# xshazwar/noize-job

Measured on AMD Instinct MI355X. Metric: Mcells/s 4096^2 simplex13oct->Gauss5x17->FlowMap->Erosion; %HBM roofline @1/8GPU, higher is better.
Workload: dtype f32

## Files before the change

noize_job_amd/csrc/nz_filter.hip:

```cpp
#include <cstdlib>

#include "nz_internal.hpp"
#include "nz_chain_plan.hpp"

namespace {

constexpr int CT = 256;
constexpr int TW = 128;
__host__ __device__ constexpr int conv_hx(int H) { return (H + 3) & ~3; }
constexpr int TH = 64;

__device__ __forceinline__ int clampi(int v, int lo, int hi) { return v < lo ? lo : (v > hi ? hi : v); }

__device__ __forceinline__ int xcd_tile_index() {
    int bid = blockIdx.x;
    int nb = gridDim.x, q = nb >> 3, r = nb & 7;
    int x = bid & 7, k = bid >> 3;
    return x * q + (x < r ? x : r) + k;
}

__device__ __forceinline__ void tile_origin(const nz_geom &g, int OW, int OH, int &ox0, int &oz0) {
    int tiles_x = (g.cols + OW - 1) / OW;
    int bid = xcd_tile_index();
    int by = bid / tiles_x;
// ... 42 lines not shown
__device__ __forceinline__ void store16_sc1(float *base, size_t float_off, float4 v) {
    __amdgpu_buffer_rsrc_t r = __builtin_amdgcn_make_buffer_rsrc(base, 0, -1, 0x00020000);
    nz_v4u t = {__float_as_uint(v.x), __float_as_uint(v.y), __float_as_uint(v.z), __float_as_uint(v.w)};
    __builtin_amdgcn_raw_buffer_store_b128(t, r, (int)(float_off * 4), 0, NZ_AUX_SC1);
}
__device__ __forceinline__ float load4_sc1(const float *base, size_t float_off) {
    __amdgpu_buffer_rsrc_t r = __builtin_amdgcn_make_buffer_rsrc(const_cast<float *>(base), 0, -1, 0x00020000);
    return __uint_as_float(__builtin_amdgcn_raw_buffer_load_b32(r, (int)(float_off * 4), 0, NZ_AUX_SC1));
}
__device__ __forceinline__ void store4_sc1(float *base, size_t float_off, float v) {
    __amdgpu_buffer_rsrc_t r = __builtin_amdgcn_make_buffer_rsrc(base, 0, -1, 0x00020000);
    __builtin_amdgcn_raw_buffer_store_b32(__float_as_uint(v), r, (int)(float_off * 4), 0, NZ_AUX_SC1);
}

template <bool FAST>
__device__ __forceinline__ float tap_acc(float total, float v, float k) {
    return FAST ? __builtin_fmaf(v, k, total) : total + v * k;
}
template <bool FAST, bool SEED>
__device__ __forceinline__ float tap_first(float v, float k) {
    return FAST ? __builtin_fmaf(v, k, 0.0f) : SEED ? 0.0f + v * k : v * k;
}

template <int KS, bool UNIT, int NT, bool SC1, bool FAST, int RBT>
__device__ __forceinline__ void conv_tile(const float *__restrict__ src, float *__restrict__ dst, const nz_geom &g,
                                          const nz_kernel_taps &taps, int T, int aligned, int ox0, int oz0,
                                          float4 *s_edge_raw NZ_PB_PARAM) {
    constexpr int O = (KS - 1) / 2;
    constexpr int WN = 4 + 2 * O;
    constexpr int ZN = RBT + 2 * O;
    constexpr int TH = NT / 32 * RBT;
    static_assert(O <= RBT, "a block's window reaches into the neighbouring blocks only");
    constexpr int NBUF = conv_nbuf(O);
    float4 (*s_edge)[TH / RBT][2][O][TW / 4] = reinterpret_cast<float4 (*)[TH / RBT][2][O][TW / 4]>(s_edge_raw);

    const int tid = threadIdx.x, cg = tid & 31, rb = tid >> 5;
    const int H = T * O, HX = conv_hx(H);
    const int OW = TW - 2 * HX, OH = TH - 2 * H;
    const int lx0 = ox0 - HX, lz0 = oz0 - H;
    const int gx0 = lx0 + cg * 4, gzb = lz0 + rb * RBT;
    const bool inside = lx0 >= 0 && lx0 + TW <= g.cols && lz0 >= g.zc0 && lz0 + TH - 1 <= g.zc1;
    const bool fast = inside && aligned;
    const bool edge16 = !inside && aligned && (g.cols & 3) == 0;
    NZ_PROBE_T(0);
    NZ_PROBE(14, (unsigned long long)__builtin_amdgcn_s_getreg(4 | (0 << 6) | (31 << 11)));
    NZ_PROBE(15, (unsigned long long)__builtin_amdgcn_s_getreg(20 | (0 << 6) | (31 << 11)));

    float v[RBT][4];
    if (fast) {
#pragma unroll
        for (int r = 0; r < RBT; r++) {
            float4 t = SC1 ? load16_sc1(src, (size_t)(gzb + r) * g.pitch + gx0)
                           : *reinterpret_cast<const float4 *>(src + (size_t)(gzb + r) * g.pitch + gx0);
            v[r][0] = t.x; v[r][1] = t.y; v[r][2] = t.z; v[r][3] = t.w;
        }
// ... 8 lines not shown
            v[r][0] = t.x; v[r][1] = t.y; v[r][2] = t.z; v[r][3] = t.w;
        }
        asm volatile("; 16-byte edge loads issued" ::: "memory");
    } else {
        asm volatile("; clamped 4-byte loads of an edge tile" ::: "memory");
#pragma unroll
        for (int r = 0; r < RBT; r++) {
            size_t row = (size_t)clampi(gzb + r, g.zc0, g.zc1) * g.pitch;
#pragma unroll
            for (int e = 0; e < 4; e++) {
                const size_t off = row + clampi(gx0 + e, 0, g.cols - 1);
                v[r][e] = SC1 ? load4_sc1(src, off) : src[off];
            }
        }
    }
    if constexpr (SC1) __builtin_amdgcn_s_setprio(0);
#ifdef NZ_CONV_PROBE
    asm volatile("s_waitcnt vmcnt(0)" ::: "memory");
    NZ_PROBE_T(9);
#endif
    const int icx = g.cols - 1 - gx0 + O;
    const int iz0 = g.zc0 - gzb + O, iz1 = g.zc1 - gzb + O;

    for (int t = 0; t < T; t++) {
#pragma unroll
        for (int r = 0; r < RBT; r++) {
            float w[WN];
#pragma unroll
            for (int o = 0; o < O; o++) {
                w[o] = dpp_prev(v[r][4 - O + o]);
                w[4 + O + o] = dpp_next(v[r][o]);
            }
#pragma unroll
            for (int e = 0; e < 4; e++) w[O + e] = v[r][e];
            if (!inside) {
                if (gx0 == 0) {
#pragma unroll
                    for (int o = 0; o < O; o++) w[o] = w[O];
                }
                if (icx >= O && icx < WN - 1) {
                    float wc = w[O];
#pragma unroll
                    for (int i = O + 1; i < WN; i++) wc = (i == icx) ? w[i] : wc;
#pragma unroll
                    for (int i = O + 1; i < WN; i++) w[i] = (i > icx) ? wc : w[i];
                }
            }
#pragma unroll
            for (int e = 0; e < 4; e++) {
// ... 28 lines not shown
            for (int e = 0; e < 4; e++) z[O + r][e] = v[r][e];
        if (!inside) {
            if (iz0 > 0 && iz0 < ZN) {
#pragma unroll
                for (int e = 0; e < 4; e++) {
                    float c = z[0][e];
#pragma unroll
                    for (int i = 1; i < ZN; i++) c = (i == iz0) ? z[i][e] : c;
#pragma unroll
                    for (int i = 0; i < ZN - 1; i++) z[i][e] = (i < iz0) ? c : z[i][e];
                }
            }
            if (iz1 >= 0 && iz1 < ZN - 1) {
#pragma unroll
                for (int e = 0; e < 4; e++) {
                    float c = z[0][e];
#pragma unroll
                    for (int i = 1; i < ZN; i++) c = (i == iz1) ? z[i][e] : c;
#pragma unroll
                    for (int i = 1; i < ZN; i++) z[i][e] = (i > iz1) ? c : z[i][e];
                }
            }
        }
#pragma unroll
        for (int r = 0; r < RBT; r++) {
#pragma unroll
            for (int e = 0; e < 4; e++) {
                float total = tap_first<FAST, !UNIT>(z[r + 2 * O][e], taps.kz[0]);
#pragma unroll
                for (int kk = 1; kk < KS; kk++) total = tap_acc<FAST>(total, z[r + 2 * O - kk][e], taps.kz[kk]);
                v[r][e] = UNIT ? total : total * taps.factor;
            }
        }
        NZ_PROBE_T(1 + t);
    }

    if constexpr (UNIT && !FAST) {
#pragma unroll
        for (int r = 0; r < RBT; r++)
#pragma unroll
            for (int e = 0; e < 4; e++) v[r][e] += 0.0f;
    }

    if constexpr (SC1) __builtin_amdgcn_s_setprio(3);
    if (fast) {
#pragma unroll
        for (int r = 0; r < RBT; r++) {
            int lr = rb * RBT + r, gz = gzb + r;
// ... 13 lines not shown
                if (SC1) store16_sc1(dst, (size_t)gz * g.pitch + gx0, make_float4(v[r][0], v[r][1], v[r][2], v[r][3]));
                else *reinterpret_cast<float4 *>(dst + (size_t)gz * g.pitch + gx0) = make_float4(v[r][0], v[r][1], v[r][2], v[r][3]);
            }
        }
    } else {
        asm volatile("; guarded stores of an edge tile" ::: "memory");
#pragma unroll
        for (int r = 0; r < RBT; r++) {
            int lr = rb * RBT + r, gz = gzb + r;
            bool in = lr >= H && lr < H + OH && cg * 4 >= HX && cg * 4 < HX + OW && gz < g.or1 && gx0 < g.cols;
            if (in) {
#pragma unroll
                for (int e = 0; e < 4; e++)
                    if (gx0 + e < g.cols) {
                        if (SC1) store4_sc1(dst, (size_t)gz * g.pitch + gx0 + e, v[r][e]);
                        else dst[(size_t)gz * g.pitch + gx0 + e] = v[r][e];
                    }
            }
        }
    }
    NZ_PROBE_T(12);
}

template <int KS, bool UNIT, int NT, bool FAST, int RBT>
__global__ __launch_bounds__(NT) __attribute__((amdgpu_waves_per_eu(conv_waves(KS, NT, RBT)))) void conv_reg_kernel(const float *__restrict__ src, float *__restrict__ dst, nz_geom g,
                                                     nz_kernel_taps taps, int T, int aligned) {
    constexpr int O = (KS - 1) / 2;
    constexpr int TH = NT / 32 * RBT;
    constexpr int NBUF = conv_nbuf(O);
    __shared__ float4 s_edge[NBUF][TH / RBT][2][O][TW / 4];
    const int H = T * O, HX = conv_hx(H);
    src += blockIdx.y * g.bstride;
    dst += blockIdx.y * g.bstride;
    int ox0, oz0;
    tile_origin(g, TW - 2 * HX, TH - 2 * H, ox0, oz0);
    NZ_PB_INIT;
    conv_tile<KS, UNIT, NT, false, FAST, RBT>(src, dst, g, taps, T, aligned, ox0, oz0, &s_edge[0][0][0][0][0] NZ_PB_ARG);
}

typedef int nz_v8i __attribute__((ext_vector_type(8)));
static_assert(sizeof(nz_v8i) == sizeof(nz_chain_item) && offsetof(nz_chain_item, stride) == 28, "a record is loaded as eight dwords");
struct nz_chain {
    const nz_chain_item *items;
    unsigned epoch;
    int *flags;
    float *plane[2];
    int delay_item, delay_sleeps;
    int spin_limit;
    unsigned *err_host;
    unsigned *err_epoch;
};

template <int KS, bool UNIT, int NT, bool FAST, int RBT>
__global__ __launch_bounds__(NT) __attribute__((amdgpu_waves_per_eu(conv_waves(KS, NT, RBT)))) void conv_chain_kernel(nz_geom g, nz_kernel_taps taps,
                                                                                                                       nz_chain ch, int aligned) {
    constexpr int O = (KS - 1) / 2;
    constexpr int TH = NT / 32 * RBT;
    constexpr int NBUF = conv_nbuf(O);
    __shared__ float4 s_edge[NBUF][TH / RBT][2][O][TW / 4];
    NZ_PB_INIT;
    NZ_PROBE_T(18);
    const nz_v8i rec = *reinterpret_cast<const nz_v8i *>(ch.items + blockIdx.x);
    __builtin_amdgcn_s_setprio(3);
    const nz_chain_item it = {rec[0], rec[1], rec[2], rec[3], rec[4], rec[5], rec[6], rec[7]};
    const int l = it.tl >> 16, T = it.tl & 0xffff;
    NZ_PROBE_T(7);
    NZ_PROBE(13, ((unsigned long long)l << 32) | (unsigned)(it.item));
    {
        const int tid = threadIdx.x, dr = tid >= 6 ? 2 : tid >= 3 ? 1 : 0, dc = tid - 3 * dr;
        if (tid < 9 && dr < it.ny && dc < it.nx) {
            const int *f = ch.flags + it.dep0 + dr * it.stride + dc;
            int spins = 0;
            while ((unsigned)__hip_atomic_load(f, __ATOMIC_RELAXED, __HIP_MEMORY_SCOPE_AGENT) != ch.epoch) {
                __builtin_amdgcn_s_sleep(32);
                if (++spins > ch.spin_limit) {
                    atomicMin(ch.err_epoch, ch.epoch);
                    __threadfence();
                    __hip_atomic_store(ch.err_host, 1u, __ATOMIC_RELEASE, __HIP_MEMORY_SCOPE_SYSTEM);
                    break;
                }
            }
        }
        if (it.ny > 0) __syncthreads();
    }
    NZ_PROBE_T(8);
    if (it.item == ch.delay_item)
        for (int i = 0; i < ch.delay_sleeps; i++) __builtin_amdgcn_s_sleep(127);
    conv_tile<KS, UNIT, NT, true, FAST, RBT>(ch.plane[l & 1], ch.plane[(l + 1) & 1], g, taps, T, aligned, it.ox0, it.oz0, &s_edge[0][0][0][0][0] NZ_PB_ARG);
    asm volatile("s_waitcnt vmcnt(0)" ::: "memory");
    NZ_PROBE_T(10);
    __syncthreads();
    NZ_PROBE_T(11);
    if (threadIdx.x == 0) {
        __hip_atomic_store(&ch.flags[it.item], (int)ch.epoch, __ATOMIC_RELAXED, __HIP_MEMORY_SCOPE_AGENT);
    }
}



template <int E>
__global__ __launch_bounds__(CT) void erosion_reg_kernel(const float *__restrict__ src, float *__restrict__ dst,
                                                        nz_geom g, int aligned) {
    __shared__ float4 s_edge[TH / RB][E][TW / 4];
    constexpr float BIG = 3.40282347e+38f;
    constexpr int HX = E > 4 ? 8 : 4;
    static_assert(E >= 1 && E <= RB, "the window reaches one 8-row block / two lanes back at most");
    const int tid = threadIdx.x, cg = tid & 31, rb = tid >> 5;
    const int OW = TW - HX, OH = TH - E;
    src += blockIdx.y * g.bstride;
    dst += blockIdx.y * g.bstride;
    int ox0, oz0;
// ... 292 lines not shown
static conv_shape conv_shape_of(int ksize, const nz_geom &g) {
    if (!conv_small_grid(ksize, g)) return CONV_BIG;
    return ksize == 5 && (long long)g.cols * (g.or1 - g.or0) * g.count <= CONV_TINY_CELLS ? CONV_TINY : CONV_SMALL;
}

template <int KS, class F>
auto with_conv_shape(conv_shape sh, F &&f) {
    using std::integral_constant;
    if constexpr (KS == 5)
        if (sh == CONV_TINY) return f(integral_constant<int, CONV_TINY_NT>(), integral_constant<int, CONV_TINY_RB>());
    if (sh != CONV_BIG) return f(integral_constant<int, CONV_SMALL_NT>(), integral_constant<int, CONV_SMALL_RB>());
    return f(integral_constant<int, (KS >= 5 ? 512 : 256)>(), integral_constant<int, RB>());
}

struct conv_tiling { int x, y; };
template <int KS, int NT, int RBT>
conv_tiling conv_tiles(const nz_geom &g, int T) {
    constexpr int O = (KS - 1) / 2, RTH = NT / 32 * RBT;
    const int H = T * O, HX = conv_hx(H);
    const int OW = TW - 2 * HX, OH = RTH - 2 * H;
    return {(g.cols + OW - 1) / OW, (g.or1 - g.or0 + OH - 1) / OH};
}

template <int KS, int NT, int RBT>
int32_t launch_fused_nt(hipStream_t s, const float *src, float *dst, const nz_geom &g, const nz_kernel_taps &k, int T) {
    const conv_tiling t = conv_tiles<KS, NT, RBT>(g, T);
    const long long blocks = (long long)t.x * t.y;
    int aligned = ((reinterpret_cast<uintptr_t>(src) | reinterpret_cast<uintptr_t>(dst) | (uintptr_t)(g.pitch * 4)) & 15) == 0;
    nz_with_unit_fast(k, [&](auto unit, auto fast) {
        NZ_LAUNCH((conv_reg_kernel<KS, unit, NT, fast, RBT>), dim3((unsigned)blocks, g.count), dim3(NT), 0, s, src, dst, g, k, T, aligned);
    });
    NZ_HIP(hipGetLastError());
    return NZ_OK;
}

template <int KS>
int32_t launch_fused(hipStream_t s, const float *src, float *dst, const nz_geom &g, const nz_kernel_taps &k, int T) {
    return with_conv_shape<KS>(conv_shape_of(KS, g), [&](auto nt, auto rbt) { return launch_fused_nt<KS, nt, rbt>(s, src, dst, g, k, T); });
}

int g_chain_delay_item = -1, g_chain_delay_sleeps = 0;
int g_chain_spin_limit = 1 << 21;

template <int KS, int NT, int RBT>
int32_t launch_chain_nt(hipStream_t s, float *plane0, float *plane1, const nz_geom &g, const nz_kernel_taps &k,
                        const nz_chain_item *items, int total, int *flags, unsigned epoch, unsigned *err_host, unsigned *err_epoch) {
    nz_chain ch{};
    ch.items = items;
    ch.epoch = epoch;
    ch.flags = flags;
    ch.plane[0] = plane0;
    ch.plane[1] = plane1;
    ch.delay_item = g_chain_delay_item;
    ch.delay_sleeps = g_chain_delay_sleeps;
    ch.spin_limit = g_chain_spin_limit;
    ch.err_host = err_host;
    ch.err_epoch = err_epoch;
    int aligned = ((reinterpret_cast<uintptr_t>(plane0) | reinterpret_cast<uintptr_t>(plane1) | (uintptr_t)(g.pitch * 4)) & 15) == 0;
    nz_with_unit_fast(k, [&](auto unit, auto fast) {
        NZ_LAUNCH((conv_chain_kernel<KS, unit, NT, fast, RBT>), dim3((unsigned)total), dim3(NT), 0, s, g, k, ch, aligned);
    });
    NZ_HIP(hipGetLastError());
    return NZ_OK;
}

template <int KS>
int32_t launch_chain(hipStream_t s, float *plane0, float *plane1, const nz_geom &g, const nz_kernel_taps &k,
                     const nz_chain_item *items, int total, int *flags, unsigned epoch, unsigned *err_host, unsigned *err_epoch) {
    return with_conv_shape<KS>(conv_shape_of(KS, g), [&](auto nt, auto rbt) {
        return launch_chain_nt<KS, nt, rbt>(s, plane0, plane1, g, k, items, total, flags, epoch, err_host, err_epoch);
    });
}

}

bool nz_conv_small_grid(int ksize, const nz_geom &g) { return conv_small_grid(ksize, g); }
bool nz_conv_tiny_grid(int ksize, const nz_geom &g) { return conv_shape_of(ksize, g) == CONV_TINY; }

bool nz_conv_chain_key(int ksize, const nz_geom &g, const int *Ts, int L, nz_chain_key *key) {
    if (L < 1 || L > NZ_CHAIN_MAXL || (ksize != 3 && ksize != 5 && ksize != 7 && ksize != 9)) return false;
    for (int l = 0; l < L; l++)
        if (Ts[l] < 1 || Ts[l] > nz_conv_max_fused(ksize)) return false;
    const conv_shape sh = conv_shape_of(ksize, g);
// ... 149 lines not shown
```

noize_job_amd/csrc/nz_flow_common.hpp:

```cpp
#pragma once

#include "nz_internal.hpp"

namespace {

constexpr float TIMESTEP = 0.2f;

__device__ __forceinline__ int clampi(int v, int lo, int hi) { return v < lo ? lo : (v > hi ? hi : v); }

struct flux4 {
    float w, e, s, n;
};

__device__ __forceinline__ flux4 compute_flow(float totalHt, float water_0, float tW, float tE, float tS, float tN,
                                              flux4 old) {
    float dW = totalHt - tW, dE = totalHt - tE, dS = totalHt - tS, dN = totalHt - tN;
    flux4 f;
    f.w = fmaxf(0.0f, old.w + dW);
    f.e = fmaxf(0.0f, old.e + dE);
    f.s = fmaxf(0.0f, old.s + dS);
    f.n = fmaxf(0.0f, old.n + dN);
    float sum_ = (f.w + f.e) + (f.s + f.n);
    if (sum_ > 0.0f) {
        float K = water_0 / (sum_ * TIMESTEP);
        K = fmaxf(0.0f, fminf(1.0f, K));
        f.w *= K; f.e *= K; f.s *= K; f.n *= K;
    } else {
        f.w = 0.0f; f.e = 0.0f; f.s = 0.0f; f.n = 0.0f;
    }
    return f;
}

__device__ __forceinline__ flux4 compute_flow_nb(float totalHt, float water_0, float tW, float tE, float tS, float tN,
                                                 flux4 old) {
    float dW = totalHt - tW, dE = totalHt - tE, dS = totalHt - tS, dN = totalHt - tN;
    flux4 f;
    f.w = fmaxf(0.0f, old.w + dW);
    f.e = fmaxf(0.0f, old.e + dE);
    f.s = fmaxf(0.0f, old.s + dS);
    f.n = fmaxf(0.0f, old.n + dN);
    float sum_ = (f.w + f.e) + (f.s + f.n);
    float K = water_0 / (sum_ * TIMESTEP);
    K = fmaxf(0.0f, fminf(1.0f, K));
    f.w *= K; f.e *= K; f.s *= K; f.n *= K;
    return f;
}

__device__ __forceinline__ float update_water(float water, flux4 own, float fE_west, float fW_east, float fN_south,
                                              float fS_north) {
    float flowOUT = own.w + own.e + own.s + own.n;
    float flowIN = 0.0f;
    flowIN += fE_west;
    flowIN += fW_east;
    flowIN += fN_south;
    flowIN += fS_north;
    float ht = water + ((flowIN - flowOUT) * TIMESTEP);
    return fmaxf(0.0f, ht);
}


template <bool FAST>
__device__ __forceinline__ flux4 compute_flow_m(float totalHt, float water_0, float tW, float tE, float tS, float tN, flux4 old,
                                                bool branch_free) {
    if (!FAST) return branch_free ? compute_flow_nb(totalHt, water_0, tW, tE, tS, tN, old) : compute_flow(totalHt, water_0, tW, tE, tS, tN, old);
    float dW = totalHt - tW, dE = totalHt - tE, dS = totalHt - tS, dN = totalHt - tN;
    flux4 f;
    f.w = fmaxf(0.0f, old.w + dW);
    f.e = fmaxf(0.0f, old.e + dE);
    f.s = fmaxf(0.0f, old.s + dS);
    f.n = fmaxf(0.0f, old.n + dN);
    float sum_ = (f.w + f.e) + (f.s + f.n);
    float K = water_0 * __builtin_amdgcn_rcpf(sum_ * TIMESTEP);
    K = fmaxf(0.0f, fminf(1.0f, K));
    f.w *= K; f.e *= K; f.s *= K; f.n *= K;
    return f;
}

template <bool FAST>
__device__ __forceinline__ float update_water_m(float water, flux4 own, float fE_west, float fW_east, float fN_south,
                                                float fS_north) {
    if (!FAST) return update_water(water, own, fE_west, fW_east, fN_south, fS_north);
    float flowOUT = own.w + own.e + own.s + own.n;
    float flowIN = ((fE_west + fW_east) + fN_south) + fS_north;
    return fmaxf(0.0f, __builtin_fmaf(flowIN - flowOUT, TIMESTEP, water));
}

template <bool FAST>
__device__ __forceinline__ float velocity_norm_m(float dl, float dr, float dt, float db, float nmin, float nrange, float inv_range) {
    const float vx = (dl + dr) * 0.5f;
    const float vy = (dt + db) * 0.5f;
    if (!FAST) {
        float v = sqrtf(vx * vx + vy * vy);
        if (nrange < 1e-12f) v = 0.0f;
        return (v - nmin) / nrange;
    }
    float v = __builtin_amdgcn_sqrtf(__builtin_fmaf(vx, vx, vy * vy));
    if (nrange < 1e-12f) v = 0.0f;
    return (v - nmin) * inv_range;
}

constexpr int FT_MAX_N = 5;

}
```

noize_job_amd/csrc/nz_flow_stream.hip:

```cpp
#include <cstdlib>

#include "nz_internal.hpp"
#include "nz_flow_common.hpp"

namespace {

__device__ __forceinline__ float wave_prev0(float v) {
    return __builtin_bit_cast(float, __builtin_amdgcn_mov_dpp(__builtin_bit_cast(int, v), 0x138, 0xf, 0xf, true));
}
__device__ __forceinline__ float wave_next0(float v) {
    return __builtin_bit_cast(float, __builtin_amdgcn_mov_dpp(__builtin_bit_cast(int, v), 0x130, 0xf, 0xf, true));
}

#ifdef NZ_FLOW_PROBE
__device__ unsigned long long *nz_flow_probe_buf = nullptr;
#define NZ_FPROBE(slot, val)                                                                                        \
    do {                                                                                                            \
        if (threadIdx.x == 0 && nz_flow_probe_buf)                                                                  \
            nz_flow_probe_buf[((size_t)blockIdx.y * gridDim.x + blockIdx.x) * 8 + (slot)] = (val);                  \
    } while (0)
#else
#define NZ_FPROBE(slot, val)
#endif
constexpr int FS_WPE = 2;
// ... 50 lines not shown
        if (i == NACT - 1) ring[((t + 2) & (FS_RING - 1)) * 64] = hn;
        const bool fa = !COND || (r >= b.loF[i] && r < b.hiF[i]);
        if (fa) {
            float left = wave_prev0(st.T0[i][NC - 1]), right = wave_next0(st.T0[i][0]);
            if (XEDGE) {
                left = lane_x0 ? st.T0[i][0] : left;
                right = lane_x1 ? st.T0[i][NC - 1] : right;
            }
#pragma unroll
            for (int e = 0; e < NC; e++) {
                const float self = st.T0[i][e];
                const float tW = e == 0 ? left : st.T0[i][e > 0 ? e - 1 : 0];
                float tE = e == NC - 1 ? right : st.T0[i][e + 1 < NC ? e + 1 : e];
                if (XEDGE && NC == 2 && e == 0 && lane_x1o) tE = self;
                float tS = st.Tm[i][e], tN = Tp[e];
                if (COND) {
                    if (r <= g.zc0) tS = self;
                    if (r >= g.zc1) tN = self;
                }
                flux4 old;
                if (i == 0) old = flux4{0.0f, 0.0f, 0.0f, 0.0f};
                else old = flux4{st.FA[i > 0 ? i - 1 : 0][e][0], st.FA[i > 0 ? i - 1 : 0][e][1],
                                 st.FA[i > 0 ? i - 1 : 0][e][2], st.FA[i > 0 ? i - 1 : 0][e][3]};
                const flux4 f = compute_flow_m<FAST>(self, st.W0[i][e], tW, tE, tS, tN, old, true);
                FC[e][0] = f.w; FC[e][1] = f.e; FC[e][2] = f.s; FC[e][3] = f.n;
            }
        } else {
#pragma unroll
            for (int e = 0; e < NC; e++)
#pragma unroll
                for (int k = 0; k < 4; k++) FC[e][k] = 0.0f;
        }
        if (i > 0) {
#pragma unroll
            for (int e = 0; e < NC; e++)
#pragma unroll
                for (int k = 0; k < 4; k++) {
                    st.FA[i > 0 ? i - 1 : 0][e][k] = st.FB[i > 0 ? i - 1 : 0][e][k];
                    st.FB[i > 0 ? i - 1 : 0][e][k] = FCprev[e][k];
                }
        }
        const int rw = r - 1;
        const bool wa = !COND || (rw >= b.loW[i] && rw < b.hiW[i]);
        float Wn[NC], Tn[NC];
#pragma unroll
        for (int e = 0; e < NC; e++) Wn[e] = Tn[e] = 0.0f;
        if (wa) {
// ... 265 lines not shown
```

noize_job_amd/csrc/nz_fractal.hip:

```cpp
#include <cstdlib>

#include "nz_internal.hpp"

namespace {

__device__ __forceinline__ float fracf_(float x) { return x - floorf(x); }
__device__ __forceinline__ float lerpf_(float a, float b, float s) { return a + s * (b - a); }
__device__ __forceinline__ float stepf_(float y, float x) { return x >= y ? 1.0f : 0.0f; }
__device__ __forceinline__ float mod289f(float x) { return x - floorf(x * (1.0f / 289.0f)) * 289.0f; }
__device__ __forceinline__ float mod7f(float x) { return x - floorf(x * (1.0f / 7.0f)) * 7.0f; }
__device__ __forceinline__ float permutef(float x) { return mod289f((34.0f * x + 1.0f) * x); }

__device__ __forceinline__ float mod289i(float x) {
    return __builtin_fmaf(-floorf(x * (1.0f / 289.0f)), 289.0f, x);
}
__device__ __forceinline__ float permutei(float x) {
    return mod289i(__builtin_fmaf(34.0f, x, 1.0f) * x);
}
__device__ __forceinline__ float twice_minus_one(float f) {
    return __builtin_fmaf(2.0f, f, -1.0f);
}
__device__ __forceinline__ float taylor_inv_sqrt(float r) { return 1.79284291400159f - 0.85373472095314f * r; }
__device__ __forceinline__ float fadef(float t) { return t * t * t * (t * (t * 6.0f - 15.0f) + 10.0f); }
__device__ __forceinline__ float rectify(float v) { return (1.0f + v) / 2.0f * 1.0f; }
// ... 412 lines not shown
        t += a * e;
    } else if constexpr (SHAPE == NZ_SHAPE_RIDGED) {
        float r = rp.offset - e;
        r = r * r;
        r = r * w;
        t += a * r;
        w = fminf(fmaxf(r * rp.gain, 0.0f), 1.0f);
    }
}
template <int SHAPE>
__device__ __forceinline__ void octave_add(float &t, float &w, float a, float v, const nz_ridge_params &rp) {
    if constexpr (SHAPE == NZ_SHAPE_FBM) {
        t += a * v;
    } else {
        shape_fold<SHAPE>(t, w, a, fabsf(twice_minus_one(v)), rp);
    }
}


template <int VEC, bool FAST, int SHAPE>
__global__ __launch_bounds__(256) void fractal_simplex_tab_kernel(float *__restrict__ dst, int rows, int cols, int pitch,
                                                                 int blocks_per_row, nz_fractal_kparams p,
                                                                 const int *__restrict__ t1g,
                                                                 const float4 *__restrict__ t2g, nz_ridge_params rp) {
    __shared__ int s_t1[NZ_T1_N];
    __shared__ float4 s_t2[FAST ? 1 : NZ_T2_N];
    __shared__ float2 s_t2f[FAST ? NZ_T2_N : 1];
    if constexpr (FAST) {
        for (int i = threadIdx.x; i < NZ_T1_N; i += 256) s_t1[i] = t1g[i] >> 1;
        for (int i = threadIdx.x; i < NZ_T2_N; i += 256) {
            const float4 g = t2g[i];
            s_t2f[i] = make_float2(g.x * g.z, g.y * g.z);
        }
    } else {
        for (int i = threadIdx.x; i < NZ_T1_N; i += 256) s_t1[i] = t1g[i];
        for (int i = threadIdx.x; i < NZ_T2_N; i += 256) s_t2[i] = t2g[i];
    }
    __syncthreads();
    fractal_batch_enter(p, dst);
    int by = blockIdx.x / blocks_per_row;
    int bx = blockIdx.x - by * blocks_per_row;
    int x0 = (bx * 256 + threadIdx.x) * VEC;
    if (x0 >= cols) return;
    float xi[VEC];
#pragma unroll
    for (int c = 0; c < VEC; c++) xi[c] = ((float)(x0 + c) + p.posx) / p.noise_size;
    int zend = min(rows, (by + 1) * p.rows_per_wg);
// ... 9 lines not shown
        if (FAST && SHAPE != NZ_SHAPE_FBM && p.fmax * reach < NZ_TAB_LIMIT) {
            for (int i = 0; i < p.octaves; i++) {
                const float zV = f * zi;
#pragma unroll
                for (int c = 0; c < VEC; c++)
                    shape_fold<SHAPE>(t[c], w[c], a, fabsf(130.0f * snoise2_tab_fast(f * xi[c], zV, s_t1, s_t2f)), rp);
                detune += p.detune_rate;
                f *= (p.stepdown - detune);
                a *= p.G;
            }
        } else if (FAST && p.fmax * reach < NZ_TAB_LIMIT) {
            float bias = 0.0f;
            for (int i = 0; i < p.octaves; i++) {
                const float zV = f * zi, a65 = 65.0f * a;
#pragma unroll
                for (int c = 0; c < VEC; c++) t[c] = __builtin_fmaf(a65, snoise2_tab_fast(f * xi[c], zV, s_t1, s_t2f), t[c]);
                bias = __builtin_fmaf(0.5f, a, bias);
                detune += p.detune_rate;
                f *= (p.stepdown - detune);
                a *= p.G;
            }
#pragma unroll
            for (int c = 0; c < VEC; c++) t[c] += bias;
        } else if (p.fmax * reach < NZ_TAB_LIMIT) {
            for (int i = 0; i < p.octaves; i++) {
                float zV = f * zi;
#pragma unroll
                for (int c = 0; c < VEC; c++) {
                    float xV = f * xi[c];
                    octave_add<SHAPE>(t[c], w[c], a, rectify_half(snoise2_tab(xV, zV, s_t1, s_t2)), rp);
                }
                detune += p.detune_rate;
                f *= (p.stepdown - detune);
                a *= p.G;
            }
        } else {
            asm volatile("; guarded octave loop" ::: "memory");
            for (int i = 0; i < p.octaves; i++) {
                float zV = f * zi;
                float xV[VEC], big = fabsf(zV);
#pragma unroll
                for (int c = 0; c < VEC; c++) {
                    xV[c] = f * xi[c];
                    big = fmaxf(big, fabsf(xV[c]));
                }
                if (!FAST && big < NZ_TAB_LIMIT) {
// ... 396 lines not shown
    long long blocks = (long long)bpr * ((rows + p.rows_per_wg - 1) / p.rows_per_wg);
    if (blocks > 0x7fffffffLL) {
        nz_set_error("fractal grid too large");
        return NZ_ERR_INVALID;
    }
    NZ_LAUNCH((fractal_kernel<BASIS, VEC, SHAPE>), dim3((unsigned)blocks, count), dim3(FR_THREADS), 0, s, dst, rows,
                       cols, pitch, bpr, static_cast<const nz_fractal_kparams &>(p), reinterpret_cast<const float2 *>(d_rgrad), p.ridge);
    NZ_HIP(hipGetLastError());
    return NZ_OK;
}

template <int SHAPE>
int32_t launch_shaped(hipStream_t s, int noiseType, float *dst, int rows, int cols, int pitch, const nz_fractal_params &p,
                      const float *d_rgrad, const void *d_simplex, int count) {
    constexpr int use_tab = 1;
    if (noiseType == NZ_NOISE_SIMPLEX && use_tab && d_simplex) {
        constexpr int VEC = 2;
        int bpr = (cols + 256 * VEC - 1) / (256 * VEC);
        long long blocks = (long long)bpr * ((rows + p.rows_per_wg - 1) / p.rows_per_wg);
        const int *t1 = reinterpret_cast<const int *>(d_simplex);
        const float4 *t2 = reinterpret_cast<const float4 *>(t1 + NZ_T1_N);
        if (nz_tls_float_mode >= NZ_FLOAT_FAST)
            NZ_LAUNCH((fractal_simplex_tab_kernel<VEC, true, SHAPE>), dim3((unsigned)blocks, count), dim3(256), 0, s, dst, rows, cols,
                      pitch, bpr, static_cast<const nz_fractal_kparams &>(p), t1, t2, p.ridge);
        else
            NZ_LAUNCH((fractal_simplex_tab_kernel<VEC, false, SHAPE>), dim3((unsigned)blocks, count), dim3(256), 0, s, dst, rows, cols,
                      pitch, bpr, static_cast<const nz_fractal_kparams &>(p), t1, t2, p.ridge);
        NZ_HIP(hipGetLastError());
        return NZ_OK;
    }
    if ((noiseType == NZ_NOISE_PERLIN || noiseType == NZ_NOISE_CELLULAR) && use_tab && d_simplex) {
        const char *base = reinterpret_cast<const char *>(d_simplex) + (NZ_T1_N * 4 + NZ_T2_N * 16);
        if (noiseType == NZ_NOISE_CELLULAR) base += NZ_TB1_N * 4 + NZ_TB2_N * 8;
        const int *t1 = reinterpret_cast<const int *>(base);
        const float2 *t2 = reinterpret_cast<const float2 *>(base + NZ_TB1_N * 4);
        if (noiseType == NZ_NOISE_PERLIN) {
            constexpr int V = 4;
            int bpr = (cols + 256 * V - 1) / (256 * V);
            long long blocks = (long long)bpr * ((rows + p.rows_per_wg - 1) / p.rows_per_wg);
            NZ_LAUNCH((fractal_tab2_kernel<NZ_NOISE_PERLIN, V, SHAPE>), dim3((unsigned)blocks, count), dim3(256), 0, s, dst, rows,
                               cols, pitch, bpr, static_cast<const nz_fractal_kparams &>(p), t1, t2, p.ridge);
        } else {
            constexpr int V = 4;
            int bpr = (cols + 256 * V - 1) / (256 * V);
            long long blocks = (long long)bpr * ((rows + p.rows_per_wg - 1) / p.rows_per_wg);
            NZ_LAUNCH((fractal_tab2_kernel<NZ_NOISE_CELLULAR, V, SHAPE>), dim3((unsigned)blocks, count), dim3(256), 0, s, dst,
                               rows, cols, pitch, bpr, static_cast<const nz_fractal_kparams &>(p), t1, t2, p.ridge);
        }
        NZ_HIP(hipGetLastError());
        return NZ_OK;
// ... 69 lines not shown
```

noize_job_amd/csrc/nz_internal.hpp:

```cpp
#pragma once

#include <hip/hip_runtime.h>
#include <hip/hip_ext.h>

#include <cstdarg>
#include <cstdint>
#include <cstdio>
#include <mutex>
#include <type_traits>
#include <vector>

#include "../../include/noize_hip.h"
#include "nz_chain_plan.hpp"
#include "nz_planes.hpp"

#define NZ_HIP(expr)                                                                      \
    do {                                                                                  \
        hipError_t e_ = (expr);                                                           \
        if (e_ != hipSuccess) {                                                           \
            nz_set_error("%s failed: %s (%s:%d)", #expr, hipGetErrorString(e_), __FILE__, \
                         __LINE__);                                                       \
            return NZ_ERR_HIP;                                                            \
        }                                                                                 \
    } while (0)
// ... 73 lines not shown
    float kx[NZ_MAX_KSIZE];
    float kz[NZ_MAX_KSIZE];
    float factor;
    int ksize;
};

struct nz_fractal_kparams {
    float posx, posz;
    float noise_size;
    float G;
    float amp;
    float stepdown, detune_rate;
    float norm;
    float fmax;
    int octaves;
    const int32_t *positions = nullptr;
    size_t bstride = 0;
    int rows_per_wg = 8;
    int shape = 0;
};
struct nz_ridge_params {
    float offset = 1.0f, gain = 2.0f;
};
struct nz_fractal_params : nz_fractal_kparams {
    nz_ridge_params ridge;
};
struct nz_warp_params {
    float strength = 0.0f, scale = 1.0f;
    int octaves = 0;
    float norm = 0.0f, fmax = 0.0f;
};

struct nz_geom {
    int cols;
    int pitch;
    int rows;
    int zc0, zc1;
    int or0, or1;
    int count = 1;
    size_t bstride = 0;
};

inline nz_geom nz_geom_batch(int res, int count) {
    nz_geom g{res, res, res, 0, res - 1, 0, res};
    g.count = count;
    g.bstride = (size_t)res * res;
    return g;
}
// ... 244 lines not shown
```

noize_job_amd/csrc/nz_stages.cpp:

```cpp
#include <cmath>
#include <cstdlib>
#include <cstring>
#include <utility>
#include <vector>

#include "nz_internal.hpp"

static float calc_fractal_norm(float hurst, int octaves) {
    float G = exp2f(-hurst);
    float a = 1.0f, t = 0.0f;
    for (int i = 0; i < octaves; i++) {
        t += a * 1.0f;
        a *= G;
    }
    return t;
}

static float fractal_fmax(float stepdown, float detune, int octaves) {
    float fmax = 0.0f, f = 1.0f, det = 0.0f;
    for (int i = 0; i < octaves; i++) {
        if (!(fabsf(f) <= fmax)) fmax = fabsf(f);
        det += detune;
        f *= (stepdown - det);
    }
    return fmax;
}

static int32_t fractal_impl(nz_ctx *ctx, hipStream_t stream, int noiseType, float *dst, int rows, int cols, int pitch,
                            float hurst,
                            float amp, float stepdown, float detune, int octaves, int xpos, int zpos_first_row,
                            int noiseSize, int count = 1, size_t bstride = 0, const int32_t *positions = nullptr,
                            int shape = NZ_SHAPE_FBM, float ridgeOffset = 1.0f, float ridgeGain = 2.0f,
                            const nz_warp_params *warp = nullptr) {
    NZ_REQUIRE(dst, "src is NULL");
    NZ_REQUIRE(noiseType >= 0 && noiseType <= NZ_NOISE_DOMAIN_ROTATED_SIMPLEX, "unknown noise type %d", noiseType);
    NZ_REQUIRE(octaves >= 0, "octaves < 0");
    NZ_REQUIRE(noiseSize != 0, "noiseSize == 0");
    nz_fractal_params p;
    p.posx = (float)xpos;
    p.posz = (float)zpos_first_row;
    p.noise_size = (float)noiseSize;
    p.G = exp2f(-hurst);
    p.amp = amp;
    p.stepdown = stepdown;
    p.detune_rate = detune;
    p.norm = calc_fractal_norm(hurst, octaves);
    p.octaves = octaves;
    p.shape = shape;
    p.ridge.offset = ridgeOffset;
    p.ridge.gain = ridgeGain;
    p.fmax = fractal_fmax(stepdown, detune, octaves);
    nz_warp_params wp;
    if (warp) {
        wp = *warp;
        wp.norm = calc_fractal_norm(hurst, wp.octaves);
        wp.fmax = fractal_fmax(stepdown, detune, wp.octaves);
    }
    return nz_launch_fractal(stream, noiseType, dst, rows, cols, pitch, p, ctx->d_rgrad, ctx->d_simplex, count, bstride,
                             positions, warp ? &wp : nullptr);
}

static void gauss_coeffs(double sigma, int width, float *out) {
    int o = (width - 1) / 2;
    double w[NZ_MAX_KSIZE], sum = 0.0;
    for (int i = 0; i < width; i++) {
        double d = (double)(i - o);
        w[i] = exp(-(d * d) / (2.0 * sigma * sigma));
        sum += w[i];
    }
    for (int i = 0; i < width; i++) out[i] = (float)(w[i] / sum);
}

static int32_t filter_taps(int32_t filter, nz_kernel_taps *t) {
    memset(t, 0, sizeof *t);
// ... 1027 lines not shown
```

Measured before the change: 28200.

## Share symmetric Gauss tap products, precompute octave table, skip first-step flux add

Adds a symmetric 5-tap convolution path that computes each tap product once and reuses it for the mirrored taps in both the horizontal and vertical passes. It is picked at runtime when the kernel weights are bit-symmetric. The fractal simplex kernel now reads per-octave frequency and amplitude from a host-precomputed table in kernel arguments instead of updating them in a serial chain. Flow-map's first iteration skips adding a zero old flux. Together these aim to cut ALU work in the conv, noise and flow stages, at the cost of more template variants and larger kernel arguments.

Result: faster. 29450 (median of 6 runs) (+4.4%).

```diff
diff --git a/noize_job_amd/csrc/nz_filter.hip b/noize_job_amd/csrc/nz_filter.hip
--- a/noize_job_amd/csrc/nz_filter.hip
+++ b/noize_job_amd/csrc/nz_filter.hip
@@ -1,4 +1,5 @@
 #include <cstdlib>
+#include <cstring>
 
 #include "nz_internal.hpp"
 #include "nz_chain_plan.hpp"
@@ -88,7 +89,7 @@
     return FAST ? __builtin_fmaf(v, k, 0.0f) : SEED ? 0.0f + v * k : v * k;
 }
 
-template <int KS, bool UNIT, int NT, bool SC1, bool FAST, int RBT>
+template <int KS, bool UNIT, int NT, bool SC1, bool FAST, int RBT, bool SYM = false>
 __device__ __forceinline__ void conv_tile(const float *__restrict__ src, float *__restrict__ dst, const nz_geom &g,
                                           const nz_kernel_taps &taps, int T, int aligned, int ox0, int oz0,
                                           float4 *s_edge_raw NZ_PB_PARAM) {
@@ -97,6 +98,7 @@
     constexpr int ZN = RBT + 2 * O;
     constexpr int TH = NT / 32 * RBT;
     static_assert(O <= RBT, "a block's window reaches into the neighbouring blocks only");
+    static_assert(!SYM || (KS == 5 && !FAST), "the shared-product form is the strict 5-tap kernel's");
     constexpr int NBUF = conv_nbuf(O);
     float4 (*s_edge)[TH / RBT][2][O][TW / 4] = reinterpret_cast<float4 (*)[TH / RBT][2][O][TW / 4]>(s_edge_raw);
 
@@ -151,9 +153,56 @@
     const int icx = g.cols - 1 - gx0 + O;
     const int iz0 = g.zc0 - gzb + O, iz1 = g.zc1 - gzb + O;
 
+    float kx0 = taps.kx[0], kx1 = taps.kx[1], kx2 = taps.kx[2];
+    if constexpr (SYM) asm volatile("" : "+v"(kx0), "+v"(kx1), "+v"(kx2));
+
     for (int t = 0; t < T; t++) {
 #pragma unroll
         for (int r = 0; r < RBT; r++) {
+            if constexpr (SYM) {
+                const float l2 = dpp_prev(v[r][2]), l3 = dpp_prev(v[r][3]), n0 = dpp_next(v[r][0]), n1 = dpp_next(v[r][1]);
+                float p0[WN], p1[WN], p2[WN];
+                p0[0] = l2 * kx0;
+                p0[1] = l3 * kx0; p1[1] = l3 * kx1;
+#pragma unroll
+                for (int e = 0; e < 4; e++) {
+                    p0[2 + e] = v[r][e] * kx0; p1[2 + e] = v[r][e] * kx1; p2[2 + e] = v[r][e] * kx2;
+                }
+                p0[6] = n0 * kx0; p1[6] = n0 * kx1;
+                p0[7] = n1 * kx0;
+                if (!inside) {
+                    asm volatile("; clamps of an edge tile's products");
+                    if (gx0 == 0) {
+                        p0[0] = p0[2]; p0[1] = p0[2]; p1[1] = p1[2];
+                    }
+                    if (icx >= O && icx < WN - 1) {
+                        float c0 = p0[2], c1 = p1[2], c2 = p2[2];
+#pragma unroll
+                        for (int i = 3; i < WN; i++) {
+                            c0 = (i == icx) ? p0[i] : c0;
+                            if (i <= 6) c1 = (i == icx) ? p1[i] : c1;
+                            if (i <= 5) c2 = (i == icx) ? p2[i] : c2;
+                        }
+#pragma unroll
+                        for (int i = 3; i < WN; i++) {
+                            p0[i] = (i > icx) ? c0 : p0[i];
+                            if (i <= 6) p1[i] = (i > icx) ? c1 : p1[i];
+                            if (i <= 5) p2[i] = (i > icx) ? c2 : p2[i];
+                        }
+                    }
+                }
+#pragma unroll
+                for (int e = 0; e < 4; e++) {
+                    float total = p0[e];
+                    total += p1[e + 1];
+                    total += p2[e + 2];
+                    total += p1[e + 3];
+                    total += p0[e + 4];
+                    v[r][e] = UNIT ? total : total * taps.factor;
+                }
+                asm volatile("" : "+v"(v[r][0]), "+v"(v[r][1]), "+v"(v[r][2]), "+v"(v[r][3]));
+                continue;
+            }
             float w[WN];
 #pragma unroll
             for (int o = 0; o < O; o++) {
@@ -228,8 +277,32 @@
                 }
             }
         }
-#pragma unroll
-        for (int r = 0; r < RBT; r++) {
+        if constexpr (SYM) {
+            const float kz0 = taps.kz[0], kz1 = taps.kz[1], kz2 = taps.kz[2];
+#pragma unroll
+            for (int e = 0; e < 4; e++) {
+                float q0[ZN], q1[ZN];
+#pragma unroll
+                for (int i = 0; i < 4; i++) q0[i] = z[i][e] * kz0;
+                q1[1] = z[1][e] * kz1;
+                q1[2] = z[2][e] * kz1;
+#pragma unroll
+                for (int r = 0; r < RBT; r++) {
+                    q0[r + 4] = z[r + 4][e] * kz0;
+                    q1[r + 3] = z[r + 3][e] * kz1;
+                    float total = !UNIT ? 0.0f + q0[r + 4] : q0[r + 4];
+                    total += q1[r + 3];
+                    total += z[r + 2][e] * kz2;
+                    total += q1[r + 1];
+                    total += q0[r];
+                    v[r][e] = UNIT ? total : total * taps.factor;
+                }
+                if constexpr (RBT == 8)
+                    asm volatile("" : "+v"(v[0][e]), "+v"(v[1][e]), "+v"(v[2][e]), "+v"(v[3][e]), "+v"(v[4][e]), "+v"(v[5][e]), "+v"(v[6][e]), "+v"(v[7][e]));
+            }
+        }
+#pragma unroll
+        for (int r = 0; r < (SYM ? 0 : RBT); r++) {
 #pragma unroll
             for (int e = 0; e < 4; e++) {
                 float total = tap_first<FAST, !UNIT>(z[r + 2 * O][e], taps.kz[0]);
@@ -289,7 +362,7 @@
     NZ_PROBE_T(12);
 }
 
-template <int KS, bool UNIT, int NT, bool FAST, int RBT>
+template <int KS, bool UNIT, int NT, bool FAST, int RBT, bool SYM>
 __global__ __launch_bounds__(NT) __attribute__((amdgpu_waves_per_eu(conv_waves(KS, NT, RBT)))) void conv_reg_kernel(const float *__restrict__ src, float *__restrict__ dst, nz_geom g,
                                                      nz_kernel_taps taps, int T, int aligned) {
     constexpr int O = (KS - 1) / 2;
@@ -302,7 +375,7 @@
     int ox0, oz0;
     tile_origin(g, TW - 2 * HX, TH - 2 * H, ox0, oz0);
     NZ_PB_INIT;
-    conv_tile<KS, UNIT, NT, false, FAST, RBT>(src, dst, g, taps, T, aligned, ox0, oz0, &s_edge[0][0][0][0][0] NZ_PB_ARG);
+    conv_tile<KS, UNIT, NT, false, FAST, RBT, SYM>(src, dst, g, taps, T, aligned, ox0, oz0, &s_edge[0][0][0][0][0] NZ_PB_ARG);
 }
 
 typedef int nz_v8i __attribute__((ext_vector_type(8)));
@@ -318,7 +391,7 @@
     unsigned *err_epoch;
 };
 
-template <int KS, bool UNIT, int NT, bool FAST, int RBT>
+template <int KS, bool UNIT, int NT, bool FAST, int RBT, bool SYM>
 __global__ __launch_bounds__(NT) __attribute__((amdgpu_waves_per_eu(conv_waves(KS, NT, RBT)))) void conv_chain_kernel(nz_geom g, nz_kernel_taps taps,
                                                                                                                        nz_chain ch, int aligned) {
     constexpr int O = (KS - 1) / 2;
@@ -353,7 +426,7 @@
     NZ_PROBE_T(8);
     if (it.item == ch.delay_item)
         for (int i = 0; i < ch.delay_sleeps; i++) __builtin_amdgcn_s_sleep(127);
-    conv_tile<KS, UNIT, NT, true, FAST, RBT>(ch.plane[l & 1], ch.plane[(l + 1) & 1], g, taps, T, aligned, it.ox0, it.oz0, &s_edge[0][0][0][0][0] NZ_PB_ARG);
+    conv_tile<KS, UNIT, NT, true, FAST, RBT, SYM>(ch.plane[l & 1], ch.plane[(l + 1) & 1], g, taps, T, aligned, it.ox0, it.oz0, &s_edge[0][0][0][0][0] NZ_PB_ARG);
     asm volatile("s_waitcnt vmcnt(0)" ::: "memory");
     NZ_PROBE_T(10);
     __syncthreads();
@@ -692,13 +765,27 @@
     return {(g.cols + OW - 1) / OW, (g.or1 - g.or0 + OH - 1) / OH};
 }
 
+static bool conv_sym(const nz_kernel_taps &k) {
+    static const int env = getenv("NZ_CONV_SYM") ? atoi(getenv("NZ_CONV_SYM")) : 1;
+    if (env == 0 || k.ksize != 5) return false;
+    return memcmp(&k.kx[0], &k.kx[4], 4) == 0 && memcmp(&k.kx[1], &k.kx[3], 4) == 0 && memcmp(&k.kz[0], &k.kz[4], 4) == 0 &&
+           memcmp(&k.kz[1], &k.kz[3], 4) == 0;
+}
+
 template <int KS, int NT, int RBT>
 int32_t launch_fused_nt(hipStream_t s, const float *src, float *dst, const nz_geom &g, const nz_kernel_taps &k, int T) {
     const conv_tiling t = conv_tiles<KS, NT, RBT>(g, T);
     const long long blocks = (long long)t.x * t.y;
     int aligned = ((reinterpret_cast<uintptr_t>(src) | reinterpret_cast<uintptr_t>(dst) | (uintptr_t)(g.pitch * 4)) & 15) == 0;
+    const bool sym = conv_sym(k);
     nz_with_unit_fast(k, [&](auto unit, auto fast) {
-        NZ_LAUNCH((conv_reg_kernel<KS, unit, NT, fast, RBT>), dim3((unsigned)blocks, g.count), dim3(NT), 0, s, src, dst, g, k, T, aligned);
+        if constexpr (KS == 5 && !fast) {
+            if (sym) {
+                NZ_LAUNCH((conv_reg_kernel<KS, unit, NT, fast, RBT, true>), dim3((unsigned)blocks, g.count), dim3(NT), 0, s, src, dst, g, k, T, aligned);
+                return;
+            }
+        }
+        NZ_LAUNCH((conv_reg_kernel<KS, unit, NT, fast, RBT, false>), dim3((unsigned)blocks, g.count), dim3(NT), 0, s, src, dst, g, k, T, aligned);
     });
     NZ_HIP(hipGetLastError());
     return NZ_OK;
@@ -727,8 +814,15 @@
     ch.err_host = err_host;
     ch.err_epoch = err_epoch;
     int aligned = ((reinterpret_cast<uintptr_t>(plane0) | reinterpret_cast<uintptr_t>(plane1) | (uintptr_t)(g.pitch * 4)) & 15) == 0;
+    const bool sym = conv_sym(k);
     nz_with_unit_fast(k, [&](auto unit, auto fast) {
-        NZ_LAUNCH((conv_chain_kernel<KS, unit, NT, fast, RBT>), dim3((unsigned)total), dim3(NT), 0, s, g, k, ch, aligned);
+        if constexpr (KS == 5 && !fast) {
+            if (sym) {
+                NZ_LAUNCH((conv_chain_kernel<KS, unit, NT, fast, RBT, true>), dim3((unsigned)total), dim3(NT), 0, s, g, k, ch, aligned);
+                return;
+            }
+        }
+        NZ_LAUNCH((conv_chain_kernel<KS, unit, NT, fast, RBT, false>), dim3((unsigned)total), dim3(NT), 0, s, g, k, ch, aligned);
     });
     NZ_HIP(hipGetLastError());
     return NZ_OK;
diff --git a/noize_job_amd/csrc/nz_flow_common.hpp b/noize_job_amd/csrc/nz_flow_common.hpp
--- a/noize_job_amd/csrc/nz_flow_common.hpp
+++ b/noize_job_amd/csrc/nz_flow_common.hpp
@@ -11,6 +11,9 @@
 struct flux4 {
     float w, e, s, n;
 };
+
+template <bool FIRST>
+__device__ __forceinline__ float flux_sum(float old, float d) { return FIRST ? d : old + d; }
 
 __device__ __forceinline__ flux4 compute_flow(float totalHt, float water_0, float tW, float tE, float tS, float tN,
                                               flux4 old) {
@@ -31,14 +34,15 @@
     return f;
 }
 
+template <bool FIRST = false>
 __device__ __forceinline__ flux4 compute_flow_nb(float totalHt, float water_0, float tW, float tE, float tS, float tN,
                                                  flux4 old) {
     float dW = totalHt - tW, dE = totalHt - tE, dS = totalHt - tS, dN = totalHt - tN;
     flux4 f;
-    f.w = fmaxf(0.0f, old.w + dW);
-    f.e = fmaxf(0.0f, old.e + dE);
-    f.s = fmaxf(0.0f, old.s + dS);
-    f.n = fmaxf(0.0f, old.n + dN);
+    f.w = fmaxf(0.0f, flux_sum<FIRST>(old.w, dW));
+    f.e = fmaxf(0.0f, flux_sum<FIRST>(old.e, dE));
+    f.s = fmaxf(0.0f, flux_sum<FIRST>(old.s, dS));
+    f.n = fmaxf(0.0f, flux_sum<FIRST>(old.n, dN));
     float sum_ = (f.w + f.e) + (f.s + f.n);
     float K = water_0 / (sum_ * TIMESTEP);
     K = fmaxf(0.0f, fminf(1.0f, K));
@@ -59,10 +63,10 @@
 }
 
 
-template <bool FAST>
+template <bool FAST, bool FIRST = false>
 __device__ __forceinline__ flux4 compute_flow_m(float totalHt, float water_0, float tW, float tE, float tS, float tN, flux4 old,
                                                 bool branch_free) {
-    if (!FAST) return branch_free ? compute_flow_nb(totalHt, water_0, tW, tE, tS, tN, old) : compute_flow(totalHt, water_0, tW, tE, tS, tN, old);
+    if (!FAST) return branch_free ? compute_flow_nb<FIRST>(totalHt, water_0, tW, tE, tS, tN, old) : compute_flow(totalHt, water_0, tW, tE, tS, tN, old);
     float dW = totalHt - tW, dE = totalHt - tE, dS = totalHt - tS, dN = totalHt - tN;
     flux4 f;
     f.w = fmaxf(0.0f, old.w + dW);
@@ -79,9 +83,9 @@
 template <bool FAST>
 __device__ __forceinline__ float update_water_m(float water, flux4 own, float fE_west, float fW_east, float fN_south,
                                                 float fS_north) {
-    if (!FAST) return update_water(water, own, fE_west, fW_east, fN_south, fS_north);
     float flowOUT = own.w + own.e + own.s + own.n;
     float flowIN = ((fE_west + fW_east) + fN_south) + fS_north;
+    if (!FAST) return fmaxf(0.0f, water + ((flowIN - flowOUT) * TIMESTEP));
     return fmaxf(0.0f, __builtin_fmaf(flowIN - flowOUT, TIMESTEP, water));
 }
 
diff --git a/noize_job_amd/csrc/nz_flow_stream.hip b/noize_job_amd/csrc/nz_flow_stream.hip
--- a/noize_job_amd/csrc/nz_flow_stream.hip
+++ b/noize_job_amd/csrc/nz_flow_stream.hip
@@ -96,7 +96,8 @@
                 if (i == 0) old = flux4{0.0f, 0.0f, 0.0f, 0.0f};
                 else old = flux4{st.FA[i > 0 ? i - 1 : 0][e][0], st.FA[i > 0 ? i - 1 : 0][e][1],
                                  st.FA[i > 0 ? i - 1 : 0][e][2], st.FA[i > 0 ? i - 1 : 0][e][3]};
-                const flux4 f = compute_flow_m<FAST>(self, st.W0[i][e], tW, tE, tS, tN, old, true);
+                const flux4 f = i == 0 ? compute_flow_m<FAST, !FAST>(self, st.W0[i][e], tW, tE, tS, tN, old, true)
+                                       : compute_flow_m<FAST>(self, st.W0[i][e], tW, tE, tS, tN, old, true);
                 FC[e][0] = f.w; FC[e][1] = f.e; FC[e][2] = f.s; FC[e][3] = f.n;
             }
         } else {
diff --git a/noize_job_amd/csrc/nz_fractal.hip b/noize_job_amd/csrc/nz_fractal.hip
--- a/noize_job_amd/csrc/nz_fractal.hip
+++ b/noize_job_amd/csrc/nz_fractal.hip
@@ -458,7 +458,8 @@
 __global__ __launch_bounds__(256) void fractal_simplex_tab_kernel(float *__restrict__ dst, int rows, int cols, int pitch,
                                                                  int blocks_per_row, nz_fractal_kparams p,
                                                                  const int *__restrict__ t1g,
-                                                                 const float4 *__restrict__ t2g, nz_ridge_params rp) {
+                                                                 const float4 *__restrict__ t2g, nz_ridge_params rp,
+                                                                 nz_octave_table oct) {
     __shared__ int s_t1[NZ_T1_N];
     __shared__ float4 s_t2[FAST ? 1 : NZ_T2_N];
     __shared__ float2 s_t2f[FAST ? NZ_T2_N : 1];
@@ -514,6 +515,19 @@
             }
 #pragma unroll
             for (int c = 0; c < VEC; c++) t[c] += bias;
+        } else if (p.fmax * reach < NZ_TAB_LIMIT && oct.n > 0) {
+            float fn = oct.f[0], an = oct.a[0];
+            for (int i = 0; i < oct.n; i++) {
+                f = fn; a = an;
+                const int nx = min(i + 1, NZ_OCT_TAB - 1);
+                fn = oct.f[nx]; an = oct.a[nx];
+                float zV = f * zi;
+#pragma unroll
+                for (int c = 0; c < VEC; c++) {
+                    float xV = f * xi[c];
+                    octave_add<SHAPE>(t[c], w[c], a, rectify_half(snoise2_tab(xV, zV, s_t1, s_t2)), rp);
+                }
+            }
         } else if (p.fmax * reach < NZ_TAB_LIMIT) {
             for (int i = 0; i < p.octaves; i++) {
                 float zV = f * zi;
@@ -956,10 +970,10 @@
         const float4 *t2 = reinterpret_cast<const float4 *>(t1 + NZ_T1_N);
         if (nz_tls_float_mode >= NZ_FLOAT_FAST)
             NZ_LAUNCH((fractal_simplex_tab_kernel<VEC, true, SHAPE>), dim3((unsigned)blocks, count), dim3(256), 0, s, dst, rows, cols,
-                      pitch, bpr, static_cast<const nz_fractal_kparams &>(p), t1, t2, p.ridge);
+                      pitch, bpr, static_cast<const nz_fractal_kparams &>(p), t1, t2, p.ridge, p.oct);
         else
             NZ_LAUNCH((fractal_simplex_tab_kernel<VEC, false, SHAPE>), dim3((unsigned)blocks, count), dim3(256), 0, s, dst, rows, cols,
-                      pitch, bpr, static_cast<const nz_fractal_kparams &>(p), t1, t2, p.ridge);
+                      pitch, bpr, static_cast<const nz_fractal_kparams &>(p), t1, t2, p.ridge, p.oct);
         NZ_HIP(hipGetLastError());
         return NZ_OK;
     }
diff --git a/noize_job_amd/csrc/nz_internal.hpp b/noize_job_amd/csrc/nz_internal.hpp
--- a/noize_job_amd/csrc/nz_internal.hpp
+++ b/noize_job_amd/csrc/nz_internal.hpp
@@ -119,8 +119,14 @@
 struct nz_ridge_params {
     float offset = 1.0f, gain = 2.0f;
 };
+constexpr int NZ_OCT_TAB = 16;
+struct nz_octave_table {
+    float f[NZ_OCT_TAB], a[NZ_OCT_TAB];
+    int n = 0;
+};
 struct nz_fractal_params : nz_fractal_kparams {
     nz_ridge_params ridge;
+    nz_octave_table oct;
 };
 struct nz_warp_params {
     float strength = 0.0f, scale = 1.0f;
diff --git a/noize_job_amd/csrc/nz_stages.cpp b/noize_job_amd/csrc/nz_stages.cpp
--- a/noize_job_amd/csrc/nz_stages.cpp
+++ b/noize_job_amd/csrc/nz_stages.cpp
@@ -24,6 +24,20 @@
         f *= (stepdown - det);
     }
     return fmax;
+}
+
+static void fractal_octave_table(float amp, float G, float stepdown, float detune, int octaves, nz_octave_table *t) {
+    *t = nz_octave_table{};
+    if (octaves < 1 || octaves > NZ_OCT_TAB) return;
+    float f = 1.0f, a = amp, det = 0.0f;
+    for (int i = 0; i < NZ_OCT_TAB; i++) {
+        t->f[i] = f;
+        t->a[i] = a;
+        det += detune;
+        f *= (stepdown - det);
+        a *= G;
+    }
+    t->n = octaves;
 }
 
 static int32_t fractal_impl(nz_ctx *ctx, hipStream_t stream, int noiseType, float *dst, int rows, int cols, int pitch,
@@ -50,6 +64,7 @@
     p.ridge.offset = ridgeOffset;
     p.ridge.gain = ridgeGain;
     p.fmax = fractal_fmax(stepdown, detune, octaves);
+    fractal_octave_table(amp, p.G, stepdown, detune, octaves, &p.oct);
     nz_warp_params wp;
     if (warp) {
         wp = *warp;
```
